# VinAIResearch/LFM

Measured on AMD Instinct MI355X. Metric: images/sec, higher is better.
Workload: dtype f16; 1 GPU; DiT-L/2 celeb256 f8 (4x32x32 latents), batch 64/GPU, 50-step Euler (torchdiffeq grid) + f8 VAE decode to 256x256 + uint8 NHWC; 2 batches in flight on 2 HIP streams (same weights, own scratch); per_gpu_batch=64, global_batch=64, h2d_of_latents=inside the timed step, nfe=50, batches_in_flight=2

## Files before the change

### include/lfm_hip.h

```cpp
#ifndef LFM_HIP_H
#define LFM_HIP_H
#include <stddef.h>
#include <stdint.h>

#ifdef __cplusplus
extern "C" {
#endif

typedef void* lfm_stream_t;

#define LFM_OK 0
#define LFM_ERR_SHAPE (-1)
#define LFM_ERR_ALIGN (-2)
#define LFM_ERR_WORKSPACE (-3)
#define LFM_ERR_LAUNCH (-4)
#define LFM_ERR_ARG (-5)

const char* lfm_strerror(int code);
#define LFM_ABI_VERSION 4
int lfm_abi_version(void);

typedef struct lfm_dit_shape {
  int depth;
  int hidden;
// ... 51 lines not shown
#define LFM_CALL_ON 2
#define LFM_CALL_GEMM_SELECT(which) ((which) + 1)

size_t lfm_dit_workspace_bytes(const lfm_dit_shape* shape, int max_batch);

int lfm_dit_forward(const lfm_dit_shape* shape, const lfm_dit_weights* w, void* workspace, size_t workspace_bytes,
                    const lfm_dit_call* call, lfm_stream_t stream);

#define LFM_PLAN_FOLDED_LN 1
#define LFM_PLAN_FUSED_QKV_ATTENTION 2
int lfm_dit_plan(const lfm_dit_shape* shape, const lfm_dit_call* call, int* plan_out);

size_t lfm_dit_cond_table_bytes(const lfm_dit_shape* shape, int n_times);
int lfm_dit_cond_table_build(const lfm_dit_shape* shape, const lfm_dit_weights* w, void* workspace, size_t workspace_bytes, int batch, const float* t_values,
                             int n_times, void* table, size_t table_bytes, lfm_stream_t stream);

int lfm_gemm_f16(const void* A, long lda, const void* W, long ldw, void* C, long ldc, int M, int N, int K, const float* bias,
                 int epilogue, const float* gate, long gate_stride, int tokens, lfm_stream_t stream);

int lfm_gemm_qkv_f16(const void* A, long lda, const void* W, long ldw, void* Q, void* K_out, void* Vt, int M, int D, int K,
                     const float* bias, int head_dim, int tokens, lfm_stream_t stream);

int lfm_gemm_select(int which);
int lfm_gemm_plan(int M, int N, int K, int batch, int caps);

int lfm_profile_fc1(int enable);
int lfm_profile_blocks_read(float* host_ms_out, int max_n);
#define LFM_OPT_FOLD_LN 1
#define LFM_OPT_GEMM_V6 2
#define LFM_OPT_SKINNY_GEMM 4
#define LFM_OPT_ATTENTION_STREAM 5
#define LFM_OPT_FUSED_QKV_ATTENTION 6
#define LFM_OPT_UNET_ATTENTION_STREAM 7
int lfm_set_option(int key, int value);
int lfm_dit_call_settings(const lfm_dit_call* call, int* gemm_select_out, int* fold_ln_out);

int lfm_clock_probe(int blocks, int iters, unsigned long long* ticks_out, lfm_stream_t stream);

#ifdef LFM_MEASURE
int lfm_gemm_trace_read(unsigned long long* host_out, int n_per_group);
int lfm_attention_trace_read(unsigned long long* host_out, int n);
int lfm_attention_wg_trace_read(unsigned long long* host_out, int n_wg);
int lfm_dit_chk_arm(const void* workspace);
int lfm_dit_chk_read(unsigned long long* host_out, int n);
#endif
int lfm_profile_fc1_read(float* host_ms_out, int max_n);

int lfm_ln_modulate(const float* X, void* A, int M, int D, int tokens, const float* shift, const float* scale, long mod_stride,
                    lfm_stream_t stream);

int lfm_dit_attention(const void* Q, const void* K, const void* Vt, void* O, int batch, int heads, int T, lfm_stream_t stream);
int lfm_dit_attention_hd(const void* Q, const void* K, const void* Vt, void* O, int batch, int heads, int head_dim, int T,
                         lfm_stream_t stream);
int lfm_attention_plan(int batch, int heads, int head_dim, int T);

typedef struct lfm_vae_resnet {
  const float* n1_g; const float* n1_b; const void* c1_w; const float* c1_b;
  const float* n2_g; const float* n2_b; const void* c2_w; const float* c2_b;
  const void* sc_w; const float* sc_b;
  int cin, cout;
} lfm_vae_resnet;

typedef struct lfm_vae_weights {
  const float* pq_w; const float* pq_b;
  const float* cin_w; const float* cin_b;
  lfm_vae_resnet mid[2];
// ... 93 lines not shown
```

### lfm_amd/csrc/conv_halo_kernel.h

```cpp
#pragma once
#include "gemm256h_kernel.h"

#define CH_HALO_PIX_PAD 336
#define CH_HALO_BYTES (CH_HALO_PIX_PAD * 64)
#define CH_W_BYTES (128 * 64)
#define CH_RING_OFF (2 * CH_HALO_BYTES)
#define CH_LDS_BYTES (CH_RING_OFF + 3 * CH_W_BYTES)

template <int V>
struct ch_ic {
  static constexpr int value = V;
};

template <class Epi, class = void>
struct epi_has_finish_slab {
  static constexpr bool value = false;
};
template <class Epi>
struct epi_has_finish_slab<Epi, decltype((void)&Epi::finish_slab)> {
  static constexpr bool value = true;
};

template <class Epi, int UPS>
__global__ __launch_bounds__(256, 2) void conv3x3_halo_kernel(const half_t* __restrict__ in, const half_t* __restrict__ zeros,
                                                               const half_t* __restrict__ Wt, long ldw, int H, int W, int Cin, int tiles_x,
                                                               int tiles_per_img, int total_wg, int nb, Epi epi, int stag) {
  extern __shared__ __attribute__((aligned(16))) char smem[];
  const int tid = threadIdx.x, lane = tid & 63, wave = __builtin_amdgcn_readfirstlane(tid >> 6);
  const int wm = wave >> 1, wn = wave & 1;
#ifdef LFM_MEASURE
  lfm_stagger_start(stag);
#endif
  int l = blockIdx.x;
  if ((total_wg & 7) == 0) l = (l & 7) * (total_wg >> 3) + (l >> 3);
  const int t = l / nb, n0 = (l - t * nb) * 128;
  const int img = t / tiles_per_img, rem = t - img * tiles_per_img, ty = rem / tiles_x, tx = rem - ty * tiles_x;
  const int y0 = ty * 16, x0 = tx * 16;
  const int nh = Cin >> 5;
  const int Hs = H >> UPS, Ws = W >> UPS;
  const half_t* inimg = in + (size_t)img * Hs * Ws * Cin;

  int hoff[6];
#pragma unroll
  for (int k = 0; k < 6; ++k) {
    const int slot = (k * 4 + wave) * 64 + lane, p = slot >> 2, ch = slot & 3;
    const int hy = p / 18, hx = p - hy * 18, iy = y0 - 1 + hy, ix = x0 - 1 + hx;
    const bool ok = p < 324 && (unsigned)iy < (unsigned)H && (unsigned)ix < (unsigned)W;
    hoff[k] = ok ? ((iy >> UPS) * Ws + (ix >> UPS)) * Cin + ((ch ^ ((p >> 1) & 2)) << 3) : -1;
  }
  auto issue_halo = [&](int h, int hb) {
#pragma unroll
    for (int k = 0; k < 6; ++k) {
      const int widx = k * 4 + wave;
      if (widx < 21) {
        int o = hoff[k];
        asm volatile("" : "+v"(o));
        glds16(o >= 0 ? inimg + o + h * 32 : zeros, smem + hb * CH_HALO_BYTES + widx * 1024);
      }
    }
  };
  const half_t* wsrc[2];
#pragma unroll
  for (int k = 0; k < 2; ++k) wsrc[k] = Wt + (long)(n0 + k * 64 + wave * 16 + (lane >> 2)) * ldw + (((lane & 3) ^ ((lane >> 3) & 2)) << 3);
  auto issue_w = [&](int h, int tap, int rs) {
    const int koff = tap * Cin + h * 32;
#pragma unroll
    for (int k = 0; k < 2; ++k) glds16(wsrc[k] + koff, smem + CH_RING_OFF + rs * CH_W_BYTES + (k * 4 + wave) * 1024);
  };

  const int r = lane & 15, q = lane >> 4, pl = wm * 144 + r;
  int abase[8];
#pragma unroll
  for (int c7 = 0; c7 < 8; ++c7) abase[c7] = pl * 64 + ((q ^ ((((pl & 7) + c7) >> 1) & 2)) << 4);
  const int wbase = (wn * 64 + r) * 64 + ((q ^ ((r >> 1) & 2)) << 4);

  f32x4_t acc[8][4];
#pragma unroll
  for (int i = 0; i < 8; ++i)
#pragma unroll
    for (int j = 0; j < 4; ++j) acc[i][j] = (f32x4_t){0.f, 0.f, 0.f, 0.f};
  half8_t af[8], bf[4];
  auto lds_read = [&](half8_t& dst, int addr, auto OFFC) {
    constexpr int OFF = decltype(OFFC)::value;
    asm volatile("ds_read_b128 %0, %1 offset:%2" : "=v"(dst) : "v"(addr), "n"(OFF) : "memory");
  };

#define CH_LGKM(n) asm volatile("s_waitcnt lgkmcnt(" #n ")" ::: "memory")
  auto slab = [&](auto HBC, auto TAPC, int h) {
    constexpr int HB = decltype(HBC)::value, TAP = decltype(TAPC)::value, RS = TAP % 3;
    const bool more_h = h + 1 < nh;
    if (TAP == 8 && !more_h) asm volatile("s_waitcnt vmcnt(0)" ::: "memory");
    else if ((TAP == 1 || TAP == 2) && more_h) asm volatile("s_waitcnt vmcnt(7)" ::: "memory");
    else asm volatile("s_waitcnt vmcnt(2)" ::: "memory");
    G256_BARRIER();
    {
      constexpr int T2 = (TAP + 2) % 9;
      const int h2 = h + (TAP + 2 >= 9 ? 1 : 0);
      if (h2 < nh) issue_w(h2, T2, (RS + 2) % 3);
      if (TAP == 0 && more_h) issue_halo(h + 1, HB ^ 1);
    }
    __builtin_amdgcn_sched_barrier(0);
    constexpr int WOFF = CH_RING_OFF + RS * CH_W_BYTES;
    lds_read(bf[0], wbase, ch_ic<WOFF>{});
    lds_read(bf[1], wbase, ch_ic<WOFF + 1024>{});
    lds_read(bf[2], wbase, ch_ic<WOFF + 2048>{});
    lds_read(bf[3], wbase, ch_ic<WOFF + 3072>{});
    constexpr int DY = TAP / 3, DX = TAP % 3;
#define CH_AREAD(i)                                                               \
  {                                                                               \
    constexpr int C = ((i) + DY) * 18 + DX;                                       \
    lds_read(af[i], abase[C & 7], ch_ic<HB * CH_HALO_BYTES + C * 64>{});          \
  }
    CH_AREAD(0) CH_AREAD(1) CH_AREAD(2) CH_AREAD(3) CH_AREAD(4) CH_AREAD(5) CH_AREAD(6) CH_AREAD(7)
#undef CH_AREAD
    __builtin_amdgcn_sched_barrier(0);
#pragma unroll
    for (int i = 0; i < 8; ++i) {
      if (i == 0) CH_LGKM(7);
      else if (i == 1) CH_LGKM(6);
      else if (i == 2) CH_LGKM(5);
      else if (i == 3) CH_LGKM(4);
      else if (i == 4) CH_LGKM(3);
      else if (i == 5) CH_LGKM(2);
      else if (i == 6) CH_LGKM(1);
      else CH_LGKM(0);
      __builtin_amdgcn_sched_barrier(0);
#pragma unroll
      for (int j = 0; j < 4; ++j) acc[i][j] = __builtin_amdgcn_mfma_f32_16x16x32_f16(bf[j], af[i], acc[i][j], 0, 0, 0);
      __builtin_amdgcn_sched_barrier(0);
    }
  };
#undef CH_LGKM

  issue_halo(0, 0);
  issue_w(0, 0, 0);
  issue_w(0, 1, 1);
  for (int h = 0; h < nh; h += 2) {
    slab(ch_ic<0>{}, ch_ic<0>{}, h);
    slab(ch_ic<0>{}, ch_ic<1>{}, h);
    slab(ch_ic<0>{}, ch_ic<2>{}, h);
    slab(ch_ic<0>{}, ch_ic<3>{}, h);
    slab(ch_ic<0>{}, ch_ic<4>{}, h);
    slab(ch_ic<0>{}, ch_ic<5>{}, h);
    slab(ch_ic<0>{}, ch_ic<6>{}, h);
    slab(ch_ic<0>{}, ch_ic<7>{}, h);
    slab(ch_ic<0>{}, ch_ic<8>{}, h);
    slab(ch_ic<1>{}, ch_ic<0>{}, h + 1);
    slab(ch_ic<1>{}, ch_ic<1>{}, h + 1);
    slab(ch_ic<1>{}, ch_ic<2>{}, h + 1);
    slab(ch_ic<1>{}, ch_ic<3>{}, h + 1);
    slab(ch_ic<1>{}, ch_ic<4>{}, h + 1);
    slab(ch_ic<1>{}, ch_ic<5>{}, h + 1);
    slab(ch_ic<1>{}, ch_ic<6>{}, h + 1);
    slab(ch_ic<1>{}, ch_ic<7>{}, h + 1);
    slab(ch_ic<1>{}, ch_ic<8>{}, h + 1);
  }
  G256_BARRIER();

  char* scr = smem + wave * (32 * 272);
  const int rrow = lane >> 3, rcol = lane & 7, n = n0 + wn * 64 + rcol * 8;
#pragma unroll
  for (int I = 0; I < 4; ++I) {
#pragma unroll
    for (int h2 = 0; h2 < 2; ++h2)
#pragma unroll
      for (int j = 0; j < 4; ++j) *(f32x4_t*)(scr + (h2 * 16 + r) * 272 + (j * 16 + q * 4) * 4) = acc[2 * I + h2][j];
    asm volatile("s_waitcnt lgkmcnt(0)" ::: "memory");
    f32x4 lo[4], hi[4];
    int m[4];
    typename Epi::Aux al[4], ah[4];
#pragma unroll
    for (int ps = 0; ps < 4; ++ps) {
      const int rb = ps * 8 + rrow;
      lo[ps] = *(const f32x4*)(scr + rb * 272 + rcol * 32);
      hi[ps] = *(const f32x4*)(scr + rb * 272 + rcol * 32 + 16);
      m[ps] = (img * H + y0 + wm * 8 + 2 * I + (rb >> 4)) * W + x0 + (rb & 15);
      al[ps] = epi.load(m[ps], n);
      ah[ps] = epi.load(m[ps], n + 4);
    }
#pragma unroll
    for (int ps = 0; ps < 4; ++ps) epi.store8(m[ps], n, lo[ps], hi[ps], al[ps], ah[ps]);
    asm volatile("s_waitcnt lgkmcnt(0)" ::: "memory");
  }
  if constexpr (epi_has_finish_slab<Epi>::value) epi.finish_slab(img, rem * 2 + wm, n0 + wn * 64, lane);
}

static inline bool conv3x3_halo_takes(int n, int H, int W, int Cin, int Cout) {
  if (n <= 0 || (H & 15) || (W & 15) || (Cin & 63) || (Cout & 127)) return false;
  if ((long)n * H * W >= (1L << 31) || (long)H * W * Cin >= (1L << 31)) return false;
  const long total = (long)n * (W / 16) * (H / 16) * (Cout / 128);
  return !((total < 256 && !(lfm_gemm_debug_flags() & LFM_DBG_CONV_HALO_SMALL)) || total >= (1L << 31));
}
template <int UPS, class Epi>
static inline int launch_conv3x3_halo(const half_t* in, const half_t* zeros, const half_t* Wt, int n, int H, int W, int Cin, int Cout, const Epi& epi,
                                      hipStream_t st) {
  if (!conv3x3_halo_takes(n, H, W, Cin, Cout)) return 1;
  const int tiles_x = W / 16, tiles_per_img = tiles_x * (H / 16), nb = Cout / 128;
  const long total = (long)n * tiles_per_img * nb;
  if (((uintptr_t)in | (uintptr_t)Wt | (uintptr_t)zeros) & 15) return LFM_ERR_ALIGN;
  if (!lfm_kernel_lds<&conv3x3_halo_kernel<Epi, UPS>>(CH_LDS_BYTES)) return LFM_ERR_LAUNCH;
  hipLaunchKernelGGL((conv3x3_halo_kernel<Epi, UPS>), dim3((unsigned)total), dim3(256), CH_LDS_BYTES, st, in, zeros, Wt, 9L * Cin, H, W, Cin, tiles_x,
                     tiles_per_img, (int)total, nb, epi, lfm_stagger_ticks());
  LFM_CHECK_LAUNCH();
  return LFM_OK;
}

#define CHO_W_BYTES (9 * 16 * 64)
#define CHO_BUF_BYTES (CH_HALO_BYTES + CHO_W_BYTES)
#define CHO_LDS_BYTES (2 * CHO_BUF_BYTES)

template <class Epi>
__global__ __launch_bounds__(256, 2) void conv3x3_halo_out_kernel(const half_t* __restrict__ in, const half_t* __restrict__ zeros,
                                                                   const half_t* __restrict__ w4, int H, int W, int Cin, int tiles_x, int tiles_per_img,
                                                                   int total_tiles, Epi epi) {
  extern __shared__ __attribute__((aligned(16))) char smem[];
  const int tid = threadIdx.x, lane = tid & 63, wave = __builtin_amdgcn_readfirstlane(tid >> 6);
  int t = blockIdx.x;
  if ((total_tiles & 7) == 0) t = (t & 7) * (total_tiles >> 3) + (t >> 3);
  const int img = t / tiles_per_img, rem = t - img * tiles_per_img, ty = rem / tiles_x, tx = rem - ty * tiles_x;
  const int y0 = ty * 16, x0 = tx * 16;
  const int nh = Cin >> 5;
  const half_t* inimg = in + (size_t)img * H * W * Cin;
  int hoff[6];
#pragma unroll
  for (int k = 0; k < 6; ++k) {
    const int slot = (k * 4 + wave) * 64 + lane, p = slot >> 2, ch = slot & 3;
    const int hy = p / 18, hx = p - hy * 18, iy = y0 - 1 + hy, ix = x0 - 1 + hx;
    const bool ok = p < 324 && (unsigned)iy < (unsigned)H && (unsigned)ix < (unsigned)W;
    hoff[k] = ok ? (iy * W + ix) * Cin + ((ch ^ ((p >> 1) & 2)) << 3) : -1;
  }
  int woff[3];
#pragma unroll
  for (int k = 0; k < 3; ++k) {
    const int slot = (k * 4 + wave) * 64 + lane, tr = slot >> 2, ch = slot & 3, tap = tr >> 4, row = tr & 15;
    woff[k] = (row < 4 && tap < 9) ? row * 9 * Cin + tap * Cin + ((ch ^ ((row >> 1) & 2)) << 3) : -1;
// ... 71 lines not shown
```

### lfm_amd/csrc/debug_flags.h

```cpp
#pragma once

constexpr int LFM_DBG_GEMM_NO_EPILOGUE = 4;
constexpr int LFM_DBG_GEMM_SETPRIO = 8;
constexpr int LFM_DBG_GEMM_GM8 = 32;
constexpr int LFM_DBG_GEMM_GM2 = 64;
constexpr int LFM_DBG_GEMM_NO_XCD_REMAP = 128;
constexpr int LFM_DBG_GEMM_GM4 = 256;
constexpr int LFM_DBG_GEMM_NO_SPLITK = 512;
constexpr int LFM_DBG_GEMM_STORE8 = 1024;
constexpr int LFM_DBG_GEMM_PARITY_PRIO = 2048;
constexpr int LFM_DBG_GEMM_NEVER_V4 = 4096;
constexpr int LFM_DBG_GEMM_ALWAYS_V4 = 8192;
constexpr int LFM_DBG_GEMM_SPLITK128 = 65536;
constexpr int LFM_DBG_GEMM_ABL_SHIFT = 21;
constexpr int LFM_DBG_GEMM_ABL_MASK = 15;
constexpr int LFM_DBG_GEMM_OPT_SHIFT = 25;
constexpr int LFM_DBG_GEMM_OPT_MASK = 3;

constexpr int LFM_DBG_TRACE_GEMM = 2;
constexpr int LFM_DBG_TRACE_NO_STORES = 131072;
constexpr int LFM_DBG_TRACE_COL_SHIFT = 21;
constexpr int LFM_DBG_TRACE_COL_MASK = 15;

constexpr int LFM_DBG_ATT_WIDE = 256;
// ... 2 lines not shown

constexpr int LFM_DBG_QKV_TRACE = 2;
constexpr int LFM_DBG_QKV_NO_VT_WRITES = 262144;
constexpr int LFM_DBG_QKV_NO_QK_WRITES = 524288;
constexpr int LFM_DBG_QKV_PER_ITEM = 4194304;
constexpr int LFM_DBG_QKV_NO_KEY_LOOP = 33554432;
constexpr int LFM_DBG_QKV_TWO_KTILES = 67108864;

constexpr int LFM_DBG_LN_STORE8 = 32768;
constexpr int LFM_DBG_LN_BPERMUTE = 65536;
constexpr int LFM_DBG_LN_FOUR_ROWS = 262144;
constexpr int LFM_DBG_LN_TWO_ROWS = 524288;

constexpr int LFM_DBG_DIT_FINAL_ROUND1 = 1048576;
constexpr int LFM_DBG_DIT_PATCH_ROUND1 = 2097152;

constexpr int LFM_DBG_CONV_IMPLICIT_GEMM = 8388608;
constexpr int LFM_DBG_CONV_HALO_SMALL = 16777216;

constexpr int LFM_DBG_VAE_SEPARATE_STATS = 4194304;

constexpr int LFM_DBG_UNET_CONV_IN_SCALAR = 1;
constexpr int LFM_DBG_UNET_ATT_VALU = 16;
constexpr int LFM_DBG_UNET_GN_ROWS = 16384;

int lfm_gemm_selected();
int lfm_gemm_debug_flags();
int lfm_gemm_selected_v1_ok();
int lfm_gemm_prefers_v4(int M, int N, int K);
int lfm_gemm_v6_default();
int lfm_stagger_ticks();
int lfm_attention_stream_enabled();
int lfm_unet_attention_stream_mode();
```

### lfm_amd/csrc/dit.hip

```cpp
#include <mutex>

#include "../../include/lfm_hip.h"
#include "gemm_dispatch.h"
#include "gemm_skinny_kernel.h"
#include "gemm_sq64_kernel.h"
#include "qkv_attention_kernel.h"

typedef std::atomic<int> Opt;
static inline int opt_get(const Opt& o) { return o.load(std::memory_order_relaxed); }
static inline void opt_set(Opt& o, int v) { o.store(v, std::memory_order_relaxed); }
static struct {
  Opt gemm_sel{0}, gemm_dbg{0};
  Opt fold_ln{1};
  Opt v6{0};
  Opt skinny{1};
  Opt stagger{0};
  Opt att_stream{1};
  Opt fused_qkv{1};
  Opt unet_att_stream{1};
} g_def;
static thread_local int tl_sel_set = 0, tl_gemm_sel = 0, tl_gemm_dbg = 0;
static thread_local int tl_fold = 0;
static inline int gemm_sel() { return tl_sel_set ? tl_gemm_sel : opt_get(g_def.gemm_sel); }
static inline int gemm_dbg() { return tl_sel_set ? tl_gemm_dbg : opt_get(g_def.gemm_dbg); }
static inline int opt_fold_ln() { return tl_fold ? (tl_fold == LFM_CALL_ON ? 1 : 0) : opt_get(g_def.fold_ln); }
int lfm_gemm_selected() { return gemm_sel(); }
int lfm_gemm_debug_flags() { return gemm_dbg(); }
int lfm_gemm_selected_v1_ok() { return gemm_sel() < 2 && !(gemm_dbg() & LFM_DBG_GEMM_NO_SPLITK); }
int lfm_gemm_prefers_v4(int M, int N, int K) {
  (void)M;
  (void)N;
  (void)K;
  if (gemm_dbg() & LFM_DBG_GEMM_NEVER_V4) return 0;
  if (gemm_dbg() & LFM_DBG_GEMM_ALWAYS_V4) return 1;
  return 0;
}
int lfm_gemm_v6_default() { return opt_get(g_def.v6); }
int lfm_stagger_ticks() { return opt_get(g_def.stagger); }
int lfm_attention_stream_enabled() { return opt_get(g_def.att_stream); }
int lfm_unet_attention_stream_mode() { return opt_get(g_def.unet_att_stream); }
extern "C" int lfm_gemm_plan(int M, int N, int K, int batch, int caps) { return gemm_choose(M, N, K, batch, caps); }
static inline bool gemm_select_valid(int which) {
  const int k = which & 15;
  return which >= 0 && (k == 0 || k == 1 || k == 4 || k == 5 || k == 6 || k == 7 || k == 8);
}
struct CallScope {
  int sel_set, sel, dbg, fold;
  CallScope() : sel_set(tl_sel_set), sel(tl_gemm_sel), dbg(tl_gemm_dbg), fold(tl_fold) {}
  ~CallScope() {
    tl_sel_set = sel_set;
    tl_gemm_sel = sel;
    tl_gemm_dbg = dbg;
    tl_fold = fold;
  }
};

static int call_scope_enter(const lfm_dit_call* c) {
  if (c->fold_ln < 0 || c->fold_ln > LFM_CALL_ON || c->gemm_select < 0 || (c->gemm_select && !gemm_select_valid(c->gemm_select - 1)) || c->cond_rows < 0)
    return LFM_ERR_ARG;
  if (c->fold_ln) tl_fold = c->fold_ln;
  if (c->gemm_select) {
    tl_sel_set = 1;
    tl_gemm_sel = (c->gemm_select - 1) & 15;
    tl_gemm_dbg = (c->gemm_select - 1) >> 4;
  }
  return LFM_OK;
}
extern "C" int lfm_dit_call_settings(const lfm_dit_call* call, int* gemm_select_out, int* fold_ln_out) {
  if (!call || !gemm_select_out || !fold_ln_out) return LFM_ERR_ARG;
  CallScope scope;
  const int rc = call_scope_enter(call);
  if (rc) return rc;
  *gemm_select_out = gemm_sel() | (gemm_dbg() << 4);
  *fold_ln_out = opt_fold_ln();
  return LFM_OK;
}

extern "C" int lfm_set_option(int key, int value) {
  switch (key) {
    case 1: opt_set(g_def.fold_ln, value != 0); break;
    case 2: opt_set(g_def.v6, value != 0); break;
#ifdef LFM_MEASURE
    case 3: opt_set(g_def.stagger, value > 0 ? value : 0); break;
#endif
    case 4: opt_set(g_def.skinny, value < 0 || value > 2 ? 1 : value); break;
    case 5: opt_set(g_def.att_stream, value != 0); break;
    case 6: opt_set(g_def.fused_qkv, value != 0); break;
    case 7: opt_set(g_def.unet_att_stream, value < 0 || value > 2 ? 1 : value); break;
    default: return LFM_ERR_ARG;
  }
  return LFM_OK;
}
extern "C" int lfm_gemm_select(int which) {
  if (!gemm_select_valid(which)) return LFM_ERR_ARG;
  opt_set(g_def.gemm_sel, which & 15);
  opt_set(g_def.gemm_dbg, which >> 4);
  return LFM_OK;
}

#include "dit_kernels.h"
#include "attention_kernel.h"
#include "solver_kernels.h"
#include "dit_measure.h"

static inline size_t align_up(size_t v, size_t a) { return (v + a - 1) / a * a; }

struct DitWs {
  float* X;
  half_t* A;
  half_t* A2;
  half_t* QKVH;
  float* temb;
  float* temb_h;
  half_t* c_half;
  float* mod;
  float* ones;
  float* ln_part;
  float* cen[2];
  half_t* amod;
  float* uvq;
  float* uvf;
// ... 503 lines not shown
```

### lfm_amd/csrc/vae.hip

```cpp
#include "../../include/lfm_hip.h"
#include "nhwc_common.h"

struct EpiTransposeF16 {
  half_t* Ct;
  const float* bias;
  int T, N;
  typedef f32x4 Aux;
  __device__ __forceinline__ bool direct(int) const { return true; }
  __device__ __forceinline__ Aux load(int, int n) const { return *(const f32x4*)(bias + n); }
  __device__ __forceinline__ void store(int m, int n, f32x4 v, const Aux& b) const {
    v += b;
    const int img = m / T, tok = m - img * T;
    half_t* d = Ct + ((long)img * N + n) * T + tok;
    d[0] = (half_t)v.x;
    d[T] = (half_t)v.y;
    d[2 * T] = (half_t)v.z;
    d[3 * T] = (half_t)v.w;
  }
};

struct EpiBatchF32 {
  float* C;
  long ldc;
  typedef int Aux;
// ... 124 lines not shown
  for (; p + 3 * pstride < p1; p += 4 * pstride) {
    half8_t v[4];
#pragma unroll
    for (int u = 0; u < 4; ++u) v[u] = *(const half8_t*)(x + base + (long)(p + u * pstride) * C);
#pragma unroll
    for (int u = 0; u < 4; ++u) *(half8_t*)(y + base + (long)(p + u * pstride) * C) = one(v[u]);
  }
  for (; p < p1; p += pstride) *(half8_t*)(y + base + (long)p * C) = one(*(const half8_t*)(x + base + (long)p * C));
}

__global__ __launch_bounds__(256) void softmax_rows_kernel(const float* __restrict__ S, half_t* __restrict__ P, long rows, int T, float scale_log2e) {
  const int lane = threadIdx.x & 63;
  const long r = (long)blockIdx.x * 4 + (threadIdx.x >> 6);
  if (r >= rows) return;
  const float* s = S + r * T;
  float mx = -3.0e38f;
  for (int i = lane; i < T; i += 64) mx = fmaxf(mx, s[i]);
  mx = wave_max(mx) * scale_log2e;
  float sum = 0.f;
  for (int i = lane; i < T; i += 64) sum += __builtin_amdgcn_exp2f(s[i] * scale_log2e - mx);
  const float inv = 1.0f / wave_sum(sum);
  half_t* p = P + r * T;
  for (int i = lane; i < T; i += 64) p[i] = (half_t)(__builtin_amdgcn_exp2f(s[i] * scale_log2e - mx) * inv);
}

static inline size_t a256(size_t v) { return (v + 255) / 256 * 256; }

struct VaeWs {
  half_t *b0, *b1, *b2, *b3;
  float* stats;
  float* part;
  half_t* zeros;
  float* S;
  size_t part_pairs;
  size_t total;
};

static VaeWs vae_carve(int R, int chunk, void* ws) {
  const size_t act = (size_t)chunk * (8 * R) * (8 * R) * 256 * 2;
  const size_t T = (size_t)R * R;
  size_t off = 0;
  char* base = (char*)ws;
  auto take = [&](size_t bytes) {
    char* p = base ? base + off : nullptr;
    off += a256(bytes);
    return p;
  };
  VaeWs w;
  w.b0 = (half_t*)take(act);
  w.b1 = (half_t*)take(act);
  w.b2 = (half_t*)take(act);
  w.b3 = (half_t*)take(act);
  w.stats = (float*)take((size_t)chunk * 64 * 4);
  const size_t part_conv = (size_t)(8 * R) * (8 * R) * 256 / 512, part_stats = (size_t)VGN_MAX_SLABS * 128;
  w.part_pairs = (size_t)chunk * (part_conv > part_stats ? part_conv : part_stats);
  w.part = (float*)take(w.part_pairs * 2 * 4);
  w.zeros = (half_t*)take(256);
  w.S = (float*)take((size_t)chunk * T * T * 4);
  w.total = off;
  return w;
}

extern "C" size_t lfm_vae_workspace_bytes(int R, int chunk) {
  if (R <= 0 || chunk <= 0 || (R % 8)) return 0;
  return vae_carve(R, chunk, nullptr).total;
}

#define RC(x)            \
  do {                   \
    int _rc = (x);       \
    if (_rc) return _rc; \
  } while (0)

struct VaeConv {
  const void* w;
  const float* b;
  int Cin, Cout;
  bool ups;
};

struct VaeCtx {
  VaeWs ws;
  int n;
  hipStream_t st;
  half_t *x, *t1, *t2, *t3;
  int x_slabs;
  bool chain_stats;
  void rotate(half_t*& t) {
    half_t* o = t;
    t = x;
    x = o;
// ... 7 lines not shown
};

int VaeCtx::gn(const half_t* in, half_t* y, const float* g, const float* b, int HW, int C, bool silu, int ready_slabs) const {
  if (C % 128 || 256 % (C / 8) || C > 512) return LFM_ERR_SHAPE;
  int slabs = ready_slabs, ppb = ready_slabs ? HW / ready_slabs : 0;
  if (!ready_slabs) {
    int cap = VGN_MAX_SLABS;
    if (ws.part_pairs && n * VGN_MAX_SLABS < 1024) {
      const long room = (long)(ws.part_pairs / ((size_t)n * (C / 4)));
      const long want = 1024 / n;
      cap = (int)(want < room ? want : room);
      if (cap > 512) cap = 512;
      if (cap < VGN_MAX_SLABS) cap = VGN_MAX_SLABS;
    }
    ppb = 1024;
    if (cap > VGN_MAX_SLABS) ppb = cdiv(HW, cap) > 64 ? cdiv(HW, cap) : 64;
    if (cdiv(HW, ppb) > cap) ppb = cdiv(HW, cap);
    slabs = cdiv(HW, ppb);
    hipLaunchKernelGGL(gn_stats_rows_kernel, dim3(slabs, n), dim3(256), 0, st, GnIn{in, nullptr, C, 0}, ws.part, HW, C, ppb);
    LFM_CHECK_LAUNCH();
  }
  hipLaunchKernelGGL(gn_finish_kernel, dim3(cdiv(n * 32, 4)), dim3(256), 0, st, ws.part, ws.stats, slabs, ppb, HW, C, n * 32);
  LFM_CHECK_LAUNCH();
  const int app = HW >= 4096 ? 256 : (HW >= 256 ? 64 : HW);
  if (silu) hipLaunchKernelGGL(gn_apply_kernel<true>, dim3(cdiv(HW, app), n), dim3(256), 0, st, in, y, ws.stats, g, b, HW, C, app);
  else hipLaunchKernelGGL(gn_apply_kernel<false>, dim3(cdiv(HW, app), n), dim3(256), 0, st, in, y, ws.stats, g, b, HW, C, app);
  LFM_CHECK_LAUNCH();
  return LFM_OK;
}

int VaeCtx::conv3(const half_t* in, half_t* out, const half_t* resid, int H, int W, const VaeConv& c, int* stat_slabs, int* stat_kernel) const {
  const int Cin = c.Cin, Cout = c.Cout, HW = H * W, M = n * HW;
  const half_t* w = (const half_t*)c.w;
  if (Cin % 64 || Cout % 4) return LFM_ERR_SHAPE;
  if (stat_slabs) *stat_slabs = 0;
  if (stat_kernel) *stat_kernel = 0;
  const bool stats_ok = ws.part && stat_slabs && (HW % 256) == 0 && !(((uintptr_t)out | (uintptr_t)resid) & 15) &&
                        !(lfm_gemm_debug_flags() & LFM_DBG_VAE_SEPARATE_STATS);
  const EpiResidF16 ep{out, Cout, c.b, resid};
  const EpiConvStatsF16 es{ep, ws.part, HW, 2 * (HW / 256)};
  auto left = [&](int kernel) {
    *stat_slabs = es.slabs;
    if (stat_kernel) *stat_kernel = kernel;
  };
  if (conv_halo_allowed(out, resid)) {
    auto halo = [&](const auto& e) {
      return c.ups ? launch_conv3x3_halo<1>(in, ws.zeros, w, n, H, W, Cin, Cout, e, st) : launch_conv3x3_halo<0>(in, ws.zeros, w, n, H, W, Cin, Cout, e, st);
    };
    const int rc = stats_ok ? halo(es) : halo(ep);
    if (rc == 0 && stats_ok) left(1);
    if (rc != 1) return rc;
  }
  auto gemm = [&](const auto& a) {
    const int kern = gemm_choose(M, Cout, 9 * Cin, 1, gemm_caps<std::decay_t<decltype(a)>, EpiConvStatsF16>(a, Cout, 9L * Cin));
    if (stats_ok && (kern == 4 || kern == 5) && (Cout % (kern == 4 ? 128 : 256)) == 0 && (Cout % 128) == 0 &&
        !(lfm_gemm_debug_flags() & LFM_DBG_GEMM_STORE8)) {
      left(2);
      return launch_gemm_kernel(kern, a, w, 9L * Cin, M, Cout, 9 * Cin, es, st);
    }
    return launch_gemm_auto(a, w, 9L * Cin, M, Cout, 9 * Cin, ep, st);
  };
  if (c.ups) return gemm(ASrcConv<1>{in, ws.zeros, H, W, Cin, M});
  return gemm(ASrcConv<0>{in, ws.zeros, H, W, Cin, M});
}

static int vae_test_ctx(void* workspace, size_t bytes, int n, lfm_stream_t stream, VaeCtx& c) {
  if ((uintptr_t)workspace & 255) return LFM_ERR_ALIGN;
  const size_t head = 256 + a256((size_t)n * 64 * 4);
  if (bytes < head) return LFM_ERR_WORKSPACE;
  c = VaeCtx{};
  c.ws.zeros = (half_t*)workspace;
  c.ws.stats = (float*)((char*)workspace + 256);
  c.ws.part = (float*)((char*)workspace + head);
  c.ws.part_pairs = (bytes - head) / 8;
  c.n = n;
  c.st = (hipStream_t)stream;
  return LFM_OK;
}

extern "C" int lfm_vae_groupnorm_f16(const void* x, void* y, const float* gamma, const float* beta, void* workspace, size_t workspace_bytes, int n,
                                     int HW, int C, int silu, lfm_stream_t stream) {
  if (!x || !y || !gamma || !beta || !workspace) return LFM_ERR_ARG;
  if (n <= 0 || HW <= 0 || C <= 0) return LFM_ERR_SHAPE;
  if (((uintptr_t)x | (uintptr_t)y) & 15) return LFM_ERR_ALIGN;
  VaeCtx c;
  RC(vae_test_ctx(workspace, workspace_bytes, n, stream, c));
  if (c.ws.part_pairs < (size_t)n * VGN_MAX_SLABS * (C / 4)) return LFM_ERR_WORKSPACE;
  return c.gn((const half_t*)x, (half_t*)y, gamma, beta, HW, C, silu != 0, 0);
}

extern "C" int lfm_vae_conv3x3_gn_f16(const void* in, const void* w, const float* bias, const void* resid, void* conv_out, void* y, const float* gamma,
                                      const float* beta, void* workspace, size_t workspace_bytes, int n, int H, int W, int Cin, int Cout, int ups,
                                      int silu, int* stat_slabs, int* stat_kernel, lfm_stream_t stream) {
  if (!in || !w || !bias || !conv_out || !y || !gamma || !beta || !workspace) return LFM_ERR_ARG;
  if (n <= 0 || H <= 0 || W <= 0 || (ups && ((H | W) & 1))) return LFM_ERR_SHAPE;
  if (((uintptr_t)in | (uintptr_t)w | (uintptr_t)resid | (uintptr_t)conv_out | (uintptr_t)y) & 15) return LFM_ERR_ALIGN;
  VaeCtx c;
  RC(vae_test_ctx(workspace, workspace_bytes, n, stream, c));
  const size_t conv_pairs = (size_t)n * 2 * (H * W / 256) * (Cout / 4), stat_pairs = (size_t)n * VGN_MAX_SLABS * (Cout / 4);
  if (c.ws.part_pairs < (conv_pairs > stat_pairs ? conv_pairs : stat_pairs)) return LFM_ERR_WORKSPACE;
  if (lfm_zero_async(c.ws.zeros, 256, c.st)) return LFM_ERR_LAUNCH;
  int slabs = 0, kern = 0;
  RC(c.conv3((const half_t*)in, (half_t*)conv_out, (const half_t*)resid, H, W, VaeConv{w, bias, Cin, Cout, ups != 0}, &slabs, &kern));
  RC(c.gn((const half_t*)conv_out, (half_t*)y, gamma, beta, H * W, Cout, silu != 0, slabs));
  if (stat_slabs) *stat_slabs = slabs;
  if (stat_kernel) *stat_kernel = kern;
  return LFM_OK;
}

int VaeCtx::resnet(const lfm_vae_resnet* r, int H, int W) {
  const int HW = H * W, M = n * HW;
  int mid_slabs = 0;
  RC(gn(x, t1, r->n1_g, r->n1_b, HW, r->cin, true, x_slabs));
  RC(conv3(t1, t2, nullptr, H, W, VaeConv{r->c1_w, r->c1_b, r->cin, r->cout, false}, &mid_slabs));
  RC(gn(t2, t1, r->n2_g, r->n2_b, HW, r->cout, true, mid_slabs));
  const half_t* skip = x;
  if (r->sc_w) {
    RC(launch_gemm_auto(ASrcRowMajor{x, r->cin, M, 0}, (const half_t*)r->sc_w, r->cin, M, r->cout, r->cin, EpiResidF16{t3, r->cout, r->sc_b, nullptr}, st));
    skip = t3;
  }
  x_slabs = 0;
  RC(conv3(t1, t2, skip, H, W, VaeConv{r->c2_w, r->c2_b, r->cout, r->cout, false}, chain_stats ? &x_slabs : nullptr));
  rotate(t2);
  return LFM_OK;
}

template <class W>
int VaeCtx::mid_attention(const W* w, int T) {
  const int M = n * T, C = 512;
  RC(gn(x, t1, w->at_g, w->at_b, T, C, false, x_slabs));
  half_t* Qb = t2;
  half_t* Kb = t2 + (size_t)M * C;
  half_t* Vt = t3;
// ... 210 lines not shown
```

### lfm_amd/hip.py

```python
import ctypes as C
import os

import torch

_HERE = os.path.dirname(os.path.abspath(__file__))
LIB_PATH = os.path.join(_HERE, "_lib", "liblfm_hip.so")
_lib = None


class LfmHipError(RuntimeError):
    pass


class DitShape(C.Structure):
    _fields_ = [(n, C.c_int) for n in ("depth", "hidden", "heads", "patch", "in_ch", "res", "mlp_hidden", "label_rows")]


_DIT_WEIGHT_FIELDS = ("pos_embed", "patch_w", "patch_b", "t_w0", "t_b0", "t_w2", "t_b2", "y_table", "ada_w", "ada_b",
                      "qkv_w", "qkv_b", "proj_w", "proj_b", "fc1_w", "fc1_b", "fc2_w", "fc2_b", "final_w", "final_b", "patch_w16")


class DitWeights(C.Structure):
    _fields_ = [(n, C.c_void_p) for n in _DIT_WEIGHT_FIELDS]

# ... 249 lines not shown
DBG_GEMM_OPT_SHIFT = 25
DBG_GEMM_OPT_MASK = 3
DBG_TRACE_GEMM = 2
DBG_TRACE_NO_STORES = 131072
DBG_TRACE_COL_SHIFT = 21
DBG_TRACE_COL_MASK = 15
DBG_ATT_WIDE = 256
DBG_ATT_MODE_SHIFT = 25
DBG_ATT_MODE_MASK = 3
DBG_QKV_TRACE = 2
DBG_QKV_NO_VT_WRITES = 262144
DBG_QKV_NO_QK_WRITES = 524288
DBG_QKV_PER_ITEM = 4194304
DBG_QKV_NO_KEY_LOOP = 33554432
DBG_QKV_TWO_KTILES = 67108864
DBG_LN_STORE8 = 32768
DBG_LN_BPERMUTE = 65536
DBG_LN_FOUR_ROWS = 262144
DBG_LN_TWO_ROWS = 524288
DBG_DIT_FINAL_ROUND1 = 1048576
DBG_DIT_PATCH_ROUND1 = 2097152
DBG_CONV_IMPLICIT_GEMM = 8388608
DBG_CONV_HALO_SMALL = 16777216
DBG_VAE_SEPARATE_STATS = 4194304
DBG_UNET_CONV_IN_SCALAR = 1
DBG_UNET_ATT_VALU = 16
DBG_UNET_GN_ROWS = 16384

OPT_FOLD_LN = 1
OPT_SKINNY_GEMM = 4
OPT_ATTENTION_STREAM = 5
OPT_FUSED_QKV_ATTENTION = 6
OPT_UNET_ATTENTION_STREAM = 7
OPT_GEMM_V6 = 2


def effective_clock_mhz(device=None, iters=20000):
    dev = torch.device(device or "cuda:0")
    n = torch.cuda.get_device_properties(dev).multi_processor_count
    ticks = torch.zeros(n, dtype=torch.int64, device=dev)
    for it in (200, iters):
        e0, e1 = torch.cuda.Event(enable_timing=True), torch.cuda.Event(enable_timing=True)
        e0.record(torch.cuda.current_stream(dev))
        check(lib().lfm_clock_probe(n, it, ptr(ticks), stream_ptr(dev)), "lfm_clock_probe")
        e1.record(torch.cuda.current_stream(dev))
        torch.cuda.synchronize(dev)
    ms = e0.elapsed_time(e1)
    return 2.0 * float(ticks.max()) / (ms * 1e3)


PLAN_FOLDED_LN, PLAN_FUSED_QKV_ATTENTION = 1, 2


def dit_plan(shape, batch, t_len=1, labels=False, fold_ln=0, gemm_select=0):
    call = DitCall()
    call.batch, call.t_len, call.y = int(batch), int(t_len), (1 if labels else None)
    call.fold_ln, call.gemm_select = fold_ln, gemm_select
    plan = C.c_int(-1)
    check(lib().lfm_dit_plan(C.byref(shape), C.byref(call), C.byref(plan)), "lfm_dit_plan")
    return plan.value


GEMM_CAP_V6, GEMM_CAP_FITS = 1, 2


def gemm_plan(M, N, K, batch=1, caps=GEMM_CAP_V6 | GEMM_CAP_FITS):
# ... 56 lines not shown
```

Baseline: 120.4 images/sec.

## Decompose upsample+3x3 conv into four 2x2 subpixel phase convolutions

Adds a subpixel path for the VAE nearest-upsample followed by a 3x3 conv. A small kernel folds the 3x3 weights into four phase-specific 2x2 kernels, and the halo conv then runs each phase on the low-resolution input, using 4 taps instead of 9. This removes more than half the MFMA work and the redundant reads of duplicated pixels in the upsample convs. In exchange, the weights are refolded on every call, extra workspace is needed, and summing the folded weights in fp16 slightly changes numerics. It is enabled by default through a new option.

```diff
diff --git a/include/lfm_hip.h b/include/lfm_hip.h
--- a/include/lfm_hip.h
+++ b/include/lfm_hip.h
@@ -107,6 +107,7 @@
 #define LFM_OPT_ATTENTION_STREAM 5
 #define LFM_OPT_FUSED_QKV_ATTENTION 6
 #define LFM_OPT_UNET_ATTENTION_STREAM 7
+#define LFM_OPT_VAE_SUBPIXEL 8
 int lfm_set_option(int key, int value);
 int lfm_dit_call_settings(const lfm_dit_call* call, int* gemm_select_out, int* fold_ln_out);
 
diff --git a/lfm_amd/csrc/conv_halo_kernel.h b/lfm_amd/csrc/conv_halo_kernel.h
--- a/lfm_amd/csrc/conv_halo_kernel.h
+++ b/lfm_amd/csrc/conv_halo_kernel.h
@@ -33,26 +33,41 @@
 #endif
   int l = blockIdx.x;
   if ((total_wg & 7) == 0) l = (l & 7) * (total_wg >> 3) + (l >> 3);
-  const int t = l / nb, n0 = (l - t * nb) * 128;
+  constexpr int SUB = UPS == 2;
+  constexpr int PITCH = SUB ? 17 : 18;
+  constexpr int NPIX = PITCH * PITCH;
+  constexpr int NDMA = (NPIX * 4 + 63) / 64;
+  constexpr int NPH = SUB ? 4 : 1;
+  const int npb = nb * NPH;
+  const int t = l / npb, sub = l - t * npb, phase = SUB ? sub / nb : 0, n0 = (sub - phase * nb) * 128;
+  const int pa = phase >> 1, pb = phase & 1;
   const int img = t / tiles_per_img, rem = t - img * tiles_per_img, ty = rem / tiles_x, tx = rem - ty * tiles_x;
   const int y0 = ty * 16, x0 = tx * 16;
   const int nh = Cin >> 5;
-  const int Hs = H >> UPS, Ws = W >> UPS;
+  const int Hs = H >> (UPS != 0), Ws = W >> (UPS != 0);
   const half_t* inimg = in + (size_t)img * Hs * Ws * Cin;
+  if (SUB) Wt += (long)phase * nb * 128 * ldw;
 
   int hoff[6];
 #pragma unroll
   for (int k = 0; k < 6; ++k) {
     const int slot = (k * 4 + wave) * 64 + lane, p = slot >> 2, ch = slot & 3;
-    const int hy = p / 18, hx = p - hy * 18, iy = y0 - 1 + hy, ix = x0 - 1 + hx;
-    const bool ok = p < 324 && (unsigned)iy < (unsigned)H && (unsigned)ix < (unsigned)W;
-    hoff[k] = ok ? ((iy >> UPS) * Ws + (ix >> UPS)) * Cin + ((ch ^ ((p >> 1) & 2)) << 3) : -1;
+    const int hy = p / PITCH, hx = p - hy * PITCH;
+    if (SUB) {
+      const int iy = y0 - 1 + pa + hy, ix = x0 - 1 + pb + hx;
+      const bool ok = p < NPIX && (unsigned)iy < (unsigned)Hs && (unsigned)ix < (unsigned)Ws;
+      hoff[k] = ok ? (iy * Ws + ix) * Cin + ((ch ^ ((p >> 1) & 2)) << 3) : -1;
+    } else {
+      const int iy = y0 - 1 + hy, ix = x0 - 1 + hx;
+      const bool ok = p < NPIX && (unsigned)iy < (unsigned)H && (unsigned)ix < (unsigned)W;
+      hoff[k] = ok ? ((iy >> UPS) * Ws + (ix >> UPS)) * Cin + ((ch ^ ((p >> 1) & 2)) << 3) : -1;
+    }
   }
   auto issue_halo = [&](int h, int hb) {
 #pragma unroll
     for (int k = 0; k < 6; ++k) {
       const int widx = k * 4 + wave;
-      if (widx < 21) {
+      if (widx < NDMA) {
         int o = hoff[k];
         asm volatile("" : "+v"(o));
         glds16(o >= 0 ? inimg + o + h * 32 : zeros, smem + hb * CH_HALO_BYTES + widx * 1024);
@@ -68,7 +83,7 @@
     for (int k = 0; k < 2; ++k) glds16(wsrc[k] + koff, smem + CH_RING_OFF + rs * CH_W_BYTES + (k * 4 + wave) * 1024);
   };
 
-  const int r = lane & 15, q = lane >> 4, pl = wm * 144 + r;
+  const int r = lane & 15, q = lane >> 4, pl = wm * (8 * PITCH) + r;
   int abase[8];
 #pragma unroll
   for (int c7 = 0; c7 < 8; ++c7) abase[c7] = pl * 64 + ((q ^ ((((pl & 7) + c7) >> 1) & 2)) << 4);
@@ -130,11 +145,71 @@
       __builtin_amdgcn_sched_barrier(0);
     }
   };
+  auto slab2 = [&](auto HBC, auto TAPC, int h, int& rs) {
+    constexpr int HB = decltype(HBC)::value, TAP = decltype(TAPC)::value;
+    const bool more_h = h + 1 < nh;
+    if (TAP == 3 && !more_h) asm volatile("s_waitcnt vmcnt(0)" ::: "memory");
+    else if ((TAP == 1 || TAP == 2) && more_h) asm volatile("s_waitcnt vmcnt(6)" ::: "memory");
+    else asm volatile("s_waitcnt vmcnt(2)" ::: "memory");
+    G256_BARRIER();
+    {
+      constexpr int T2 = (TAP + 2) & 3;
+      const int h2 = h + (TAP >= 2 ? 1 : 0);
+      if (h2 < nh) issue_w(h2, T2, rs == 0 ? 2 : rs - 1);
+      if (TAP == 0 && more_h) issue_halo(h + 1, HB ^ 1);
+    }
+    __builtin_amdgcn_sched_barrier(0);
+    const int wb = wbase + rs * CH_W_BYTES;
+    rs = rs == 2 ? 0 : rs + 1;
+    lds_read(bf[0], wb, ch_ic<CH_RING_OFF>{});
+    lds_read(bf[1], wb, ch_ic<CH_RING_OFF + 1024>{});
+    lds_read(bf[2], wb, ch_ic<CH_RING_OFF + 2048>{});
+    lds_read(bf[3], wb, ch_ic<CH_RING_OFF + 3072>{});
+    constexpr int DY = TAP >> 1, DX = TAP & 1;
+#define CH_AREAD(i)                                                               \
+  {                                                                               \
+    constexpr int C = ((i) + DY) * 17 + DX;                                       \
+    lds_read(af[i], abase[C & 7], ch_ic<HB * CH_HALO_BYTES + C * 64>{});          \
+  }
+    CH_AREAD(0) CH_AREAD(1) CH_AREAD(2) CH_AREAD(3) CH_AREAD(4) CH_AREAD(5) CH_AREAD(6) CH_AREAD(7)
+#undef CH_AREAD
+    __builtin_amdgcn_sched_barrier(0);
+#pragma unroll
+    for (int i = 0; i < 8; ++i) {
+      if (i == 0) CH_LGKM(7);
+      else if (i == 1) CH_LGKM(6);
+      else if (i == 2) CH_LGKM(5);
+      else if (i == 3) CH_LGKM(4);
+      else if (i == 4) CH_LGKM(3);
+      else if (i == 5) CH_LGKM(2);
+      else if (i == 6) CH_LGKM(1);
+      else CH_LGKM(0);
+      __builtin_amdgcn_sched_barrier(0);
+#pragma unroll
+      for (int j = 0; j < 4; ++j) acc[i][j] = __builtin_amdgcn_mfma_f32_16x16x32_f16(bf[j], af[i], acc[i][j], 0, 0, 0);
+      __builtin_amdgcn_sched_barrier(0);
+    }
+  };
 #undef CH_LGKM
 
   issue_halo(0, 0);
   issue_w(0, 0, 0);
   issue_w(0, 1, 1);
+  if constexpr (SUB) {
+    int rs = 0;
+    for (int h = 0; h < nh; h += 2) {
+      slab2(ch_ic<0>{}, ch_ic<0>{}, h, rs);
+      slab2(ch_ic<0>{}, ch_ic<1>{}, h, rs);
+      slab2(ch_ic<0>{}, ch_ic<2>{}, h, rs);
+      slab2(ch_ic<0>{}, ch_ic<3>{}, h, rs);
+      if (h + 1 < nh) {
+        slab2(ch_ic<1>{}, ch_ic<0>{}, h + 1, rs);
+        slab2(ch_ic<1>{}, ch_ic<1>{}, h + 1, rs);
+        slab2(ch_ic<1>{}, ch_ic<2>{}, h + 1, rs);
+        slab2(ch_ic<1>{}, ch_ic<3>{}, h + 1, rs);
+      }
+    }
+  } else
   for (int h = 0; h < nh; h += 2) {
     slab(ch_ic<0>{}, ch_ic<0>{}, h);
     slab(ch_ic<0>{}, ch_ic<1>{}, h);
@@ -174,7 +249,8 @@
       const int rb = ps * 8 + rrow;
       lo[ps] = *(const f32x4*)(scr + rb * 272 + rcol * 32);
       hi[ps] = *(const f32x4*)(scr + rb * 272 + rcol * 32 + 16);
-      m[ps] = (img * H + y0 + wm * 8 + 2 * I + (rb >> 4)) * W + x0 + (rb & 15);
+      const int py = y0 + wm * 8 + 2 * I + (rb >> 4), px = x0 + (rb & 15);
+      m[ps] = SUB ? (img * H + 2 * py + pa) * W + 2 * px + pb : (img * H + py) * W + px;
       al[ps] = epi.load(m[ps], n);
       ah[ps] = epi.load(m[ps], n + 4);
     }
@@ -182,7 +258,7 @@
     for (int ps = 0; ps < 4; ++ps) epi.store8(m[ps], n, lo[ps], hi[ps], al[ps], ah[ps]);
     asm volatile("s_waitcnt lgkmcnt(0)" ::: "memory");
   }
-  if constexpr (epi_has_finish_slab<Epi>::value) epi.finish_slab(img, rem * 2 + wm, n0 + wn * 64, lane);
+  if constexpr (epi_has_finish_slab<Epi>::value) epi.finish_slab(img, (rem * NPH + phase) * 2 + wm, n0 + wn * 64, lane);
 }
 
 static inline bool conv3x3_halo_takes(int n, int H, int W, int Cin, int Cout) {
@@ -201,6 +277,53 @@
   if (!lfm_kernel_lds<&conv3x3_halo_kernel<Epi, UPS>>(CH_LDS_BYTES)) return LFM_ERR_LAUNCH;
   hipLaunchKernelGGL((conv3x3_halo_kernel<Epi, UPS>), dim3((unsigned)total), dim3(256), CH_LDS_BYTES, st, in, zeros, Wt, 9L * Cin, H, W, Cin, tiles_x,
                      tiles_per_img, (int)total, nb, epi, lfm_stagger_ticks());
+  LFM_CHECK_LAUNCH();
+  return LFM_OK;
+}
+
+inline __global__ __launch_bounds__(256) void fold_ups_weights_kernel(const half_t* __restrict__ w, half_t* __restrict__ wf, int Cout, int Cin) {
+  const int c8 = Cin >> 3;
+  const long i = (long)blockIdx.x * 256 + threadIdx.x;
+  if (i >= 16L * Cout * c8) return;
+  const int ci = (int)(i % c8) * 8;
+  const long t = i / c8;
+  const int tap = (int)(t & 3), co = (int)((t >> 2) % Cout), ph = (int)((t >> 2) / Cout);
+  const int a = ph >> 1, b = ph & 1, r = tap >> 1, s = tap & 1;
+  const int ky0 = r ? (a ? 2 : 1) : 0, ky1 = r ? 2 : (a ? 1 : 0), kx0 = s ? (b ? 2 : 1) : 0, kx1 = s ? 2 : (b ? 1 : 0);
+  float acc[8] = {0.f, 0.f, 0.f, 0.f, 0.f, 0.f, 0.f, 0.f};
+  for (int ky = ky0; ky <= ky1; ++ky)
+    for (int kx = kx0; kx <= kx1; ++kx) {
+      const half8_t v = *(const half8_t*)(w + ((long)co * 9 + ky * 3 + kx) * Cin + ci);
+#pragma unroll
+      for (int j = 0; j < 8; ++j) acc[j] += (float)v[j];
+    }
+  half8_t o;
+#pragma unroll
+  for (int j = 0; j < 8; ++j) o[j] = (half_t)acc[j];
+  *(half8_t*)(wf + i * 8) = o;
+}
+
+static inline bool conv3x3_subpixel_takes(int n, int H, int W, int Cin, int Cout) {
+  if (n <= 0 || H <= 0 || W <= 0 || (H & 31) || (W & 31) || Cin <= 0 || (Cin & 31) || Cout <= 0 || (Cout & 127)) return false;
+  if ((long)n * H * W >= (1L << 31) || (long)(H / 2) * (W / 2) * Cin >= (1L << 31)) return false;
+  const long total = (long)n * (W / 32) * (H / 32) * 4 * (Cout / 128);
+  return !((total < 256 && !(lfm_gemm_debug_flags() & LFM_DBG_CONV_HALO_SMALL)) || total >= (1L << 31));
+}
+static inline size_t conv3x3_subpixel_wf_bytes(int Cin, int Cout) { return (size_t)16 * Cout * Cin * sizeof(half_t); }
+
+template <class Epi>
+static inline int launch_conv3x3_subpixel(const half_t* in, const half_t* zeros, const half_t* w, half_t* wf, int n, int H, int W, int Cin, int Cout,
+                                          const Epi& epi, hipStream_t st) {
+  if (!conv3x3_subpixel_takes(n, H, W, Cin, Cout)) return 1;
+  const int tiles_x = W / 32, tiles_per_img = tiles_x * (H / 32), nb = Cout / 128;
+  const long total = (long)n * tiles_per_img * 4 * nb;
+  if (((uintptr_t)in | (uintptr_t)w | (uintptr_t)wf | (uintptr_t)zeros) & 15) return LFM_ERR_ALIGN;
+  if (!lfm_kernel_lds<&conv3x3_halo_kernel<Epi, 2>>(CH_LDS_BYTES)) return LFM_ERR_LAUNCH;
+  const long fold_threads = 16L * Cout * (Cin / 8);
+  hipLaunchKernelGGL(fold_ups_weights_kernel, dim3((unsigned)((fold_threads + 255) / 256)), dim3(256), 0, st, w, wf, Cout, Cin);
+  LFM_CHECK_LAUNCH();
+  hipLaunchKernelGGL((conv3x3_halo_kernel<Epi, 2>), dim3((unsigned)total), dim3(256), CH_LDS_BYTES, st, in, zeros, (const half_t*)wf, 4L * Cin, H, W, Cin,
+                     tiles_x, tiles_per_img, (int)total, nb, epi, lfm_stagger_ticks());
   LFM_CHECK_LAUNCH();
   return LFM_OK;
 }
diff --git a/lfm_amd/csrc/debug_flags.h b/lfm_amd/csrc/debug_flags.h
--- a/lfm_amd/csrc/debug_flags.h
+++ b/lfm_amd/csrc/debug_flags.h
@@ -58,3 +58,4 @@
 int lfm_stagger_ticks();
 int lfm_attention_stream_enabled();
 int lfm_unet_attention_stream_mode();
+int lfm_vae_subpixel_enabled();
diff --git a/lfm_amd/csrc/dit.hip b/lfm_amd/csrc/dit.hip
--- a/lfm_amd/csrc/dit.hip
+++ b/lfm_amd/csrc/dit.hip
@@ -18,6 +18,7 @@
   Opt att_stream{1};
   Opt fused_qkv{1};
   Opt unet_att_stream{1};
+  Opt vae_subpixel{1};
 } g_def;
 static thread_local int tl_sel_set = 0, tl_gemm_sel = 0, tl_gemm_dbg = 0;
 static thread_local int tl_fold = 0;
@@ -39,6 +40,7 @@
 int lfm_stagger_ticks() { return opt_get(g_def.stagger); }
 int lfm_attention_stream_enabled() { return opt_get(g_def.att_stream); }
 int lfm_unet_attention_stream_mode() { return opt_get(g_def.unet_att_stream); }
+int lfm_vae_subpixel_enabled() { return opt_get(g_def.vae_subpixel); }
 extern "C" int lfm_gemm_plan(int M, int N, int K, int batch, int caps) { return gemm_choose(M, N, K, batch, caps); }
 static inline bool gemm_select_valid(int which) {
   const int k = which & 15;
@@ -87,6 +89,7 @@
     case 5: opt_set(g_def.att_stream, value != 0); break;
     case 6: opt_set(g_def.fused_qkv, value != 0); break;
     case 7: opt_set(g_def.unet_att_stream, value < 0 || value > 2 ? 1 : value); break;
+    case 8: opt_set(g_def.vae_subpixel, value != 0); break;
     default: return LFM_ERR_ARG;
   }
   return LFM_OK;
diff --git a/lfm_amd/csrc/vae.hip b/lfm_amd/csrc/vae.hip
--- a/lfm_amd/csrc/vae.hip
+++ b/lfm_amd/csrc/vae.hip
@@ -180,6 +180,8 @@
   float* part;
   half_t* zeros;
   float* S;
+  half_t* wf;
+  size_t wf_bytes;
   size_t part_pairs;
   size_t total;
 };
@@ -205,6 +207,8 @@
   w.part = (float*)take(w.part_pairs * 2 * 4);
   w.zeros = (half_t*)take(256);
   w.S = (float*)take((size_t)chunk * T * T * 4);
+  w.wf_bytes = conv3x3_subpixel_wf_bytes(512, 512);
+  w.wf = (half_t*)take(w.wf_bytes);
   w.total = off;
   return w;
 }
@@ -278,7 +282,6 @@
 int VaeCtx::conv3(const half_t* in, half_t* out, const half_t* resid, int H, int W, const VaeConv& c, int* stat_slabs, int* stat_kernel) const {
   const int Cin = c.Cin, Cout = c.Cout, HW = H * W, M = n * HW;
   const half_t* w = (const half_t*)c.w;
-  if (Cin % 64 || Cout % 4) return LFM_ERR_SHAPE;
   if (stat_slabs) *stat_slabs = 0;
   if (stat_kernel) *stat_kernel = 0;
   const bool stats_ok = ws.part && stat_slabs && (HW % 256) == 0 && !(((uintptr_t)out | (uintptr_t)resid) & 15) &&
@@ -289,6 +292,13 @@
     *stat_slabs = es.slabs;
     if (stat_kernel) *stat_kernel = kernel;
   };
+  if (c.ups && lfm_vae_subpixel_enabled() && ws.wf && ws.wf_bytes >= conv3x3_subpixel_wf_bytes(Cin, Cout) && conv_halo_allowed(out, resid)) {
+    const int rc = stats_ok ? launch_conv3x3_subpixel(in, ws.zeros, w, ws.wf, n, H, W, Cin, Cout, es, st)
+                            : launch_conv3x3_subpixel(in, ws.zeros, w, ws.wf, n, H, W, Cin, Cout, ep, st);
+    if (rc == 0 && stats_ok) left(3);
+    if (rc != 1) return rc;
+  }
+  if (Cin % 64 || Cout % 4) return LFM_ERR_SHAPE;
   if (conv_halo_allowed(out, resid)) {
     auto halo = [&](const auto& e) {
       return c.ups ? launch_conv3x3_halo<1>(in, ws.zeros, w, n, H, W, Cin, Cout, e, st) : launch_conv3x3_halo<0>(in, ws.zeros, w, n, H, W, Cin, Cout, e, st);
@@ -344,7 +354,17 @@
   VaeCtx c;
   RC(vae_test_ctx(workspace, workspace_bytes, n, stream, c));
   const size_t conv_pairs = (size_t)n * 2 * (H * W / 256) * (Cout / 4), stat_pairs = (size_t)n * VGN_MAX_SLABS * (Cout / 4);
-  if (c.ws.part_pairs < (conv_pairs > stat_pairs ? conv_pairs : stat_pairs)) return LFM_ERR_WORKSPACE;
+  const size_t need_pairs = conv_pairs > stat_pairs ? conv_pairs : stat_pairs;
+  if (c.ws.part_pairs < need_pairs) return LFM_ERR_WORKSPACE;
+  if (ups && Cin > 0 && Cout > 0) {
+    const size_t head = (size_t)((char*)c.ws.part - (char*)workspace), wfb = conv3x3_subpixel_wf_bytes(Cin, Cout);
+    const size_t wf_off = workspace_bytes >= wfb ? (workspace_bytes - wfb) & ~(size_t)255 : 0;
+    if (wf_off >= head + need_pairs * 8) {
+      c.ws.wf = (half_t*)((char*)workspace + wf_off);
+      c.ws.wf_bytes = wfb;
+      c.ws.part_pairs = (wf_off - head) / 8;
+    }
+  }
   if (lfm_zero_async(c.ws.zeros, 256, c.st)) return LFM_ERR_LAUNCH;
   int slabs = 0, kern = 0;
   RC(c.conv3((const half_t*)in, (half_t*)conv_out, (const half_t*)resid, H, W, VaeConv{w, bias, Cin, Cout, ups != 0}, &slabs, &kern));
diff --git a/lfm_amd/hip.py b/lfm_amd/hip.py
--- a/lfm_amd/hip.py
+++ b/lfm_amd/hip.py
@@ -305,6 +305,7 @@
 OPT_ATTENTION_STREAM = 5
 OPT_FUSED_QKV_ATTENTION = 6
 OPT_UNET_ATTENTION_STREAM = 7
+OPT_VAE_SUBPIXEL = 8
 OPT_GEMM_V6 = 2
 
 
```

Result: no change. 121.1 images/sec, median of 6 (+0.6%).
